# maksimt/rri_nmf

Hardware: AMD Instinct MI355X
Metric: RRI sweeps/sec and achieved HBM GB/s on dense X (n x d, rank k) (higher is better)
Workload: dtype f64

## Files before the change

rri_nmf_amd/csrc/rri_hip.hip:

```cpp
#include <hip/hip_runtime.h>
#include <dlfcn.h>
#include <rccl/rccl.h>

#include <algorithm>
#include <atomic>
#include <chrono>
#include <cmath>
#include <cstdarg>
#include <cstdio>
#include <mutex>
#include <cstdlib>
#include <cstring>
#include <string>
#include <utility>
#include <vector>

#include "rri_hip.h"
#include "rri_layout.hpp"
#include "rri_pick.hpp"
#include "rri_kernels.hpp"
#include "rri_wrri_kernels.hpp"
#include "rri_sparse_kernels.hpp"
#include "rri_onchip_kernels.hpp"

// ... 857 lines not shown
            return;
        }
        const size_t sh = resid_shmem(c);
        flavour([&](auto mk, auto we) {
            hipLaunchKernelGGL((k_resid<SX, mk, we>), dim3(nb), dim3(256), sh, c->stream, (const SX*)c->X, c->ldx, M, ldm, Mbits, ldb,
                               (const double*)c->W, c->ldw, (const double*)c->T, c->LD, (int)c->n, (int)c->d, c->k, rowobj, rowpos, E,
                               c->LD, resid_w_resident(c) ? 1 : 0, xscale(c));
        });
    }
    static void reset_row(rri_ctx* c) {
        if constexpr (!RO) {
            if (c->sparse) {
                (void)hipMemsetAsync(c->xraw, 0, (size_t)c->LD * sizeof(double), c->stream);
                hipLaunchKernelGGL((k_sp_reset_row<SX>), dim3((unsigned)std::max(1, (c->sp_max_row + 255) / 256)), dim3(256), 0,
                                   c->stream, (const i64*)c->sp_rowptr, (const int*)c->sp_col, (const SX*)c->sp_x,
                                   (const double*)c->W, c->ldw, (const double*)c->T, c->LD, c->k, (const i64*)c->itmp,
                                   c->xraw);
                if (c->sparse_x && c->uni_n > 0)
                    hipLaunchKernelGGL(k_spu_reset_row, dim3((unsigned)((c->d + 255) / 256)), dim3(256), 0, c->stream,
                                       (const int*)c->uni_rows, (int)c->uni_n, c->uni_value, (const double*)c->W, c->ldw,
                                       (const double*)c->T, c->LD, c->d, c->k, (const i64*)c->itmp, c->xraw);
                return;
            }
        }
        hipLaunchKernelGGL((k_reset_row<SX>), dim3((unsigned)((c->d + 255) / 256)), dim3(256), 0, c->stream,
                           (const SX*)c->X, c->ldx, (const double*)c->W, c->ldw, (const double*)c->T, c->LD,
                           (int)c->d, c->k, (const i64*)c->itmp, c->xraw, xscale(c));
    }
    static hipError_t set_attrs(const rri_ctx* c) {
        hipError_t e = allow_lds<k_resid<SX, false, false>>(c, 160 * 1024);
        if constexpr (!RO) {
            if (e == hipSuccess) e = allow_lds<k_resid<SX, true, true>>(c, 160 * 1024);
            if (e == hipSuccess) e = allow_lds<k_resid<SX, true, false>>(c, 160 * 1024);
            if (e == hipSuccess) e = allow_lds<k_resid<SX, false, true>>(c, 160 * 1024);
            if (e == hipSuccess) e = allow_lds<k_spx_pass<SX>>(c, SP_BLOCK_BYTES + 64);
        }
        return e;
    }
};

#define DISPATCH(c, expr)                       \
    do {                                        \
        if ((c)->dtype == RRI_F32) {            \
            typedef LaunchX<float> L;           \
            expr;                               \
        } else if ((c)->dtype == RRI_F64) {     \
            typedef LaunchX<double> L;          \
            expr;                               \
        } else {                                \
            f16_unreachable(c);                 \
        }                                       \
    } while (0)
#define DISPATCH_RO(c, expr)                    \
    do {                                        \
        if ((c)->dtype == RRI_F32) {            \
            typedef LaunchX<float> L;           \
            expr;                               \
        } else if ((c)->dtype == RRI_F64) {     \
            typedef LaunchX<double> L;          \
            expr;                               \
        } else if ((c)->dtype == RRI_F16) {     \
            typedef LaunchX<_Float16> L;        \
            expr;                               \
        } else {                                \
            typedef LaunchX<unsigned char> L;   \
            expr;                               \
        }                                       \
    } while (0)

struct LK {
    static int gpart_rows(const rri_ctx* c) { return c->gpart_n; }
    template <bool UPDATE>
    static void wcol_resid(rri_ctx* c, int t, int tn, int sweep) {
        TimedScope ts(c, 1);
        hipLaunchKernelGGL((k_wcol_resid<UPDATE>), dim3(c->nwb256), dim3(256), 0, c->stream, c->W, c->ldw, (int)c->n,
                           c->k, t, tn, (const double*)c->Ypart, c->npanels, (const double*)c->Ttpart, c->nsplit,
                           c->dwv, c->Gpart, sweep, kparams(c), c->st);
        c->gpart_n = c->nwb256;
    }
    static size_t wcol_shmem(const rri_ctx* c) { return (size_t)(2 * c->k + 2 + 256 + 64) * sizeof(double); }
    template <bool UPDATE, bool CARRY>
    static void wcol_src(rri_ctx* c, int t, int tn, int sweep, const double* ypart, int nslices) {
        TimedScope ts(c, 1);
        hipLaunchKernelGGL((k_wcol<UPDATE, CARRY>), dim3(c->nwb), dim3(256), wcol_shmem(c), c->stream, c->W, c->ldw,
                           (int)c->n, c->k, t, tn, ypart, nslices, (const double*)c->Ttpart, c->ttpart_n, c->Gpart,
                           c->XYpart + (i64)t * c->xy_stride, sweep, kparams(c), c->st);
        c->gpart_n = c->nwb;
        if (UPDATE) note_xy(c, t, c->nwb * WCOL_TILES);
    }
    static void note_xy(rri_ctx* c, int t, int rows) {
        if (t == 0) { c->xy_run = 1; c->xy_rows = rows; }
        else c->xy_run = (c->xy_run == t && c->xy_rows == rows) ? t + 1 : -1;
        c->xy_valid = c->xy_run == c->k;
    }
    template <bool UPDATE, bool CARRY>
    static void wcol(rri_ctx* c, int t, int tn, int sweep) {
        wcol_src<UPDATE, CARRY>(c, t, tn, sweep, (const double*)c->Ypart, c->npanels);
    }
    static void reduce(rri_ctx* c) {
        const int nb = (int)((c->LD + 31) / 32) + GRAM_SLICES;
        hipLaunchKernelGGL(k_reduce, dim3(nb), dim3(1024), 0, c->stream, (const double*)c->Zpart, c->LD, c->nrb,
                           (const double*)c->Gpart, gpart_rows(c), c->k, c->red, (const DevState*)c->st);
    }
    static bool light(const rri_ctx* c) { return !(c->prm.project_T_each_iter && c->prm.has_t_row_sum); }
    static void trow(rri_ctx* c, int t, int check_prev, int tprev, int sweep, bool force_final) {
        hipLaunchKernelGGL(k_trow_numer, dim3(c->ntb), dim3(128), 0, c->stream, c->T, c->LD, (int)c->d, c->k, t,
                           (const double*)c->red, c->LD, c->xraw, c->tpart, c->tpart_idx, check_prev, tprev, sweep,
                           kparams(c), c->st, resid_sched(c) ? 1 : 0, resid_sched(c) ? c->told : (double*)nullptr);
        c->tpart_n = c->ntb;
        trow_final_if_needed(c, t, sweep, force_final);
    }
    static bool small(const rri_ctx* c) { return rri::trow_small(gpart_rows(c), c->k, c->ntb32); }
    static void trow_small(rri_ctx* c, int t, int check_prev, int tprev, int sweep, bool force_final) {
        hipLaunchKernelGGL(k_trow_small, dim3(c->ntb32), dim3(1024), 0, c->stream, c->T, c->LD, (int)c->d, c->k, t,
                           (const double*)c->Zpart, c->nrb, (const double*)c->Gpart, gpart_rows(c), c->red, c->LD, c->xraw,
                           c->tpart, c->tpart_idx, check_prev, tprev, sweep, kparams(c), c->st, resid_sched(c) ? 1 : 0,
                           resid_sched(c) ? c->told : (double*)nullptr);
        c->tpart_n = c->ntb32;
        trow_final_if_needed(c, t, sweep, force_final);
    }
    static void trow_final_if_needed(rri_ctx* c, int t, int sweep, bool force_final) {
        if (!light(c) || force_final)
            hipLaunchKernelGGL(k_trow_final, dim3(1), dim3(1024), 0, c->stream, c->T, c->LD, (int)c->d, t, c->xraw,
                               (const double*)c->tpart, (const i64*)c->tpart_idx, c->tpart_n, sweep, kparams(c), c->st);
    }
    static void check_prev_only(rri_ctx* c, int tprev, int sweep, int pos) {
        hipLaunchKernelGGL(k_check_red, dim3(1), dim3(64), 0, c->stream, (const double*)c->red, c->LD, c->k, tprev,
                           sweep, pos, kparams(c), c->st);
    }
    static void tgram(rri_ctx* c, int t, int finish, int sweep) {
        c->ttpart_n = c->nsplit;
        hipLaunchKernelGGL(k_tgram, dim3(c->k, c->nsplit), dim3(256), 0, c->stream, (const double*)c->T, c->LD,
                           (int)c->d, c->k, t, c->Ttpart, (const double*)c->tpart, c->tpart_n, finish, sweep,
                           kparams(c), c->st);
    }
    static void scale_wcol(rri_ctx* c, int t) {
        hipLaunchKernelGGL(k_scale_wcol, dim3((unsigned)((c->n + 255) / 256)), dim3(256), 0, c->stream, c->W,
                           c->ldw, (int)c->n, t, (const DevState*)c->st);
    }
    static void check_wcol(rri_ctx* c, int tprev, int sweep, int pos) {
        hipLaunchKernelGGL(k_check_wcol, dim3(1), dim3(256), 0, c->stream, (const double*)c->Gpart, gpart_rows(c), c->k,
                           tprev, sweep, pos, kparams(c), c->st);
    }
    static void proj_rows(rri_ctx* c, double s, const double* svec) {
        hipLaunchKernelGGL(k_proj_rows, dim3((unsigned)((c->n + 255) / 256)), dim3(256), 0, c->stream, c->W, c->ldw, (int)c->n, c->k, s,
                           svec);
    }
    static void norms(rri_ctx* c, const double* A, i64 rows, i64 cols, i64 ld) {
        hipLaunchKernelGGL(k_norms, dim3(256), dim3(256), 0, c->stream, A, rows, cols, ld, c->normpart);
    }
    static void reset_commit(rri_ctx* c, int t) {
        const i64 m = std::max(c->n, c->d);
        hipLaunchKernelGGL(k_reset_commit, dim3((unsigned)((m + 255) / 256)), dim3(256), 0, c->stream, c->W, c->ldw,
                           c->T, c->LD, (int)c->n, (int)c->d, t, (const i64*)c->itmp, (const double*)c->xraw);
    }
    static void set_row_col(rri_ctx* c, int t, const double* trow, const double* wcolv) {
        const i64 m = std::max(c->n, c->d);
        hipLaunchKernelGGL(k_set_row_col, dim3((unsigned)((m + 255) / 256)), dim3(256), 0, c->stream, c->W, c->ldw,
                           c->T, c->LD, (int)c->n, (int)c->d, t, trow, wcolv);
    }
    static void argmax_rows(rri_ctx* c, int* out) {
        hipLaunchKernelGGL(k_argmax_rows, dim3((unsigned)((c->n + 255) / 256)), dim3(256), 0, c->stream,
                           (const double*)c->W, c->ldw, (int)c->n, c->k, out);
    }
    static void masked_sqerr(rri_ctx* c, const i64* ij, const double* vals, i64 count, double lo, double hi) {
        hipLaunchKernelGGL(k_masked_sqerr, dim3(256), dim3(256), 0, c->stream, (const double*)c->W, c->ldw,
                           (const double*)c->T, c->LD, c->k, ij, vals, count, lo, hi, c->normpart);
    }
};

void launch_convert(rri_ctx* c, int src_dtype, int dst_dtype, bool transpose, const void* src, i64 lds_, void* dst, i64 ldd,
                    i64 rows, i64 cols) {
    const i64 total = rows * cols;
    const unsigned nb = (unsigned)std::min<i64>(4096, (total + 255) / 256);
    pick_type<float, double>(src_dtype, [&](auto s) {
        typedef typename decltype(s)::type Src;
        pick_type<float, double>(dst_dtype, [&](auto d) {
            typedef typename decltype(d)::type Dst;
            pick_bool(transpose, [&](auto tr) {
                hipLaunchKernelGGL((k_convert2d<Src, Dst, tr>), dim3(nb ? nb : 1), dim3(256), 0, c->stream, (const Src*)src,
                                   lds_, (Dst*)dst, ldd, rows, cols);
            });
        });
    });
}

rri_status to_device_half(rri_ctx* c, const void* host, i64 ld, int host_dtype, void* dev, i64 ldd, i64 rows, i64 cols,
                          bool transpose) {
    if (transpose) return fail(c, RRI_ERR_INVALID, "float16 storage is for X only");
    const size_t hs = dtype_size(host_dtype);
    const i64 total = rows * cols;
    const unsigned nb = (unsigned)std::max<i64>(1, std::min<i64>(4096, (total + 255) / 256));
    DevTmp tmp, part;
    HIPCHK(c, tmp.alloc((size_t)rows * cols * hs));
    HIPCHK(c, part.alloc((size_t)nb * 3 * sizeof(double)));
// ... 739 lines not shown
    c->xy_valid = whole_last;
    c->obj_track_pending = a.track != 0;
    return true;
}

void enqueue_from(rri_ctx* c, Cursor cur) {
    if (cur.sweep < c->run_total && onchip_ok(c) && enqueue_onchip(c, cur)) return;
    if (c->until.active && cur.sweep < c->run_total) c->run_total = cur.sweep + 1;
    enqueue_range(c, cur, c->run_total);
    flush_wcheck(c, c->run_total, 0);
}

rri_status read_state(rri_ctx* c, DevState* out) {
    HIPCHK(c, hipMemcpyAsync(out, c->st, sizeof(DevState), hipMemcpyDeviceToHost, c->stream));
    HIPCHK(c, hipStreamSynchronize(c->stream));
    if (c->comm_status != RRI_OK) {
        const rri_status r = c->comm_status;
        c->comm_status = RRI_OK;
        changed(c, CH_ENDED);
        return r;
    }
    return RRI_OK;
}

rri_status status_from_halt(rri_ctx* c, const DevState& s, int32_t* sweeps_done) {
    if (s.halt == 0) {
        c->paused = false;
        if (sweeps_done) *sweeps_done = c->run_total;
        return RRI_OK;
    }
    changed(c, CH_ENDED);
    if (s.halt == HALT_EVENT_STOP) {
        c->paused = false;
        if (sweeps_done) *sweeps_done = s.halt_sweep;
        return RRI_OK;
    }
    if (s.halt > 0) {
        if (c->until.active) c->run_total = std::min(c->run_total, (s.halt == HALT_EVENT_RESET_W && s.halt_pos == 0) ? s.halt_sweep : s.halt_sweep + 1);
        c->paused = true;
        c->pending.kind = s.halt == HALT_EVENT_RESET_T ? RRI_EVENT_RESET_T : RRI_EVENT_RESET_W;
        c->pending.topic = s.halt_topic;
        c->pending.sweep = s.halt_sweep;
        c->pending.resume_topic = s.halt_pos;
        if (s.halt == HALT_EVENT_RESET_T) c->resume_at = Cursor{s.halt_sweep, s.halt_topic, 1};
        else c->resume_at = Cursor{s.halt_sweep, s.halt_pos, 0};
        if (sweeps_done) *sweeps_done = s.halt_sweep;
        return RRI_PAUSED;
    }
    c->paused = false;
    if (sweeps_done) *sweeps_done = s.halt_sweep;
    switch (s.halt) {
        case HALT_ERR_UNBOUNDED:
            return fail(c, RRI_ERR_UNBOUNDED, "Minimum objective is unbounded (topic %d)", s.halt_topic);
        case HALT_ERR_W_COL_ZERO:
            return fail(c, RRI_ERR_W_COL_ZERO, "W[:, t] sums to 0 (topic %d)", s.halt_topic);
        case HALT_ERR_NOT_IMPLEMENTED:
            return fail(c, RRI_ERR_NOT_IMPLEMENTED, "s=%g is not yet implemented", c->prm.t_row_sum);
        case HALT_ERR_GRID_SYNC:
            return fail(c, RRI_ERR_HIP, "the persistent sweep's workgroups could not synchronise (not all resident); RRI_ONCHIP=0 selects the launch-per-phase schedule");
        default:
            return fail(c, RRI_ERR_INVALID, "unknown device status %d", s.halt);
    }
}

rri_status clear_halt(rri_ctx* c) {
    HIPCHK(c, hipMemsetAsync(c->st, 0, 32, c->stream));
    return RRI_OK;
}

rri_switches read_switches() {
    rri_switches sw;
    if (const char* e = getenv("RRI_ONCHIP")) sw.onchip = atoi(e) != 0;
    if (const char* e = getenv("RRI_ONCHIP_OBJ")) sw.onchip_obj = atoi(e) != 0;
    if (const char* e = getenv("RRI_WSWEEP")) sw.wsweep = atoi(e) != 0;
    if (const char* e = getenv("RRI_OBJ_DIRECT")) sw.obj_direct = atoi(e) != 0;
    if (const char* e = getenv("RRI_WMCORR_COLS")) sw.wmcorr_cols = atoi(e) != 0;
    if (const char* e = getenv("RRI_WNW_MASK")) sw.wnw_mask = atoi(e) != 0;
    if (const char* e = getenv("RRI_PASS_ROT")) sw.pass_rot = atoi(e) & 7;
    if (const char* e = getenv("RRI_ROT_CAL")) sw.rot_cal = std::max(0, atoi(e));
    sw.rot_debug = getenv("RRI_ROT_DEBUG") != nullptr;
    if (const char* e = getenv("RRI_MASK_BITS")) sw.mask_bits = atoi(e) != 0;
    if (const char* e = getenv("RRI_PASS_CACHE_MB")) sw.pass_cache_mb = std::max(0.0, atof(e));
    if (const char* e = getenv("RRI_X_PACK")) sw.x_pack = atoi(e) != 0;
    if (const char* e = getenv("RRI_PASS_PK_GEOM")) {
        char* end = nullptr;
        sw.pk_rows = (int)std::min<long>(std::max<long>(0, strtol(e, &end, 10)), 1 << 20);
        sw.pk_il = (end && *end == 'i') ? 1 : (end && *end == 'c') ? 0 : -1;
    }
    return sw;
}

const char* sparse_data_refusal(const rri_ctx* c) {
    return c->sparse_x ? "an RRI_UNWEIGHTED_SPARSE handle keeps X as CSR: it takes its data through rri_upload_X_csr only "
                         "(no dense X, no device binding, no mask)"
                       : "a sparse-pattern handle takes its data through rri_upload_observed_csr";
}

#define REFUSE_RO(c, what)                                                                                              \
    if (ro_store((c)->dtype))                                                                                           \
        return fail((c), RRI_ERR_UNSUPPORTED, "%s is not available on an %s handle (%s stores a dense X that is only read)", what, \
                    dtype_name((c)->dtype), (c)->dtype == RRI_F16 ? "float16" : "uint8")

rri_status ready(rri_ctx* c) {
    if (!c->have_X || !c->have_W || !c->have_T || !c->have_params)
        return fail(c, RRI_ERR_INVALID, "X, W, T and params must be set before stepping");
    if (c->weighted && !c->have_M) return fail(c, RRI_ERR_INVALID, "weighted handle without a mask");
    return RRI_OK;
}

}

extern "C" {

uint32_t rri_abi_version(void) { return RRI_ABI_VERSION; }

const char* rri_last_error(const rri_ctx* ctx) { return ctx ? ctx->err.c_str() : g_create_error.c_str(); }

rri_status rri_create(rri_ctx** out, int64_t n, int64_t d, int32_t k, int32_t dtype, int32_t weighted,
                      int32_t device, void* stream) {
    if (!out) return RRI_ERR_INVALID;
    *out = nullptr;
    if (n < 1 || d < 1 || k < 1) return fail(nullptr, RRI_ERR_INVALID, "need n,d,k >= 1 (got %lld,%lld,%d)", n, d, k);
    if (dtype != RRI_F32 && dtype != RRI_F64 && dtype != RRI_F16 && dtype != RRI_U8)
        return fail(nullptr, RRI_ERR_INVALID, "dtype must be RRI_F32, RRI_F64, RRI_F16 or RRI_U8");
    if (n > 2000000000LL || d > 2000000000LL) return fail(nullptr, RRI_ERR_INVALID, "n, d must fit int32");
    if (k > RRI_MAX_K) return fail(nullptr, RRI_ERR_UNSUPPORTED, "k=%d is above the rank limit RRI_MAX_K = %d of the device path", k, RRI_MAX_K);
    int ndev = 0;
    if (hipGetDeviceCount(&ndev) != hipSuccess || ndev < 1)
        return fail(nullptr, RRI_ERR_HIP, "no HIP device available (librri_hip needs an MI355X)");
    if (device < 0 || device >= ndev) return fail(nullptr, RRI_ERR_INVALID, "device %d out of range [0,%d)", device, ndev);
    if (weighted < 0 || weighted > 4)
        return fail(nullptr, RRI_ERR_INVALID, "weighted must be RRI_UNWEIGHTED, RRI_WEIGHTED_DENSE, RRI_WEIGHTED_SPARSE, "
                                              "RRI_UNWEIGHTED_RESIDUAL or RRI_UNWEIGHTED_SPARSE");
    if (ro_store(dtype) && weighted != RRI_UNWEIGHTED) {
        static const struct { int dtype; const char *stores, *rewritten, *csr; } refusal[] = {
            {RRI_U8, "RRI_U8 stores read-only dense counts (RRI_UNWEIGHTED)", "keeps a stored residual, which counts 0..255 cannot hold",
             "keeps its values in a CSR store, which has no uint8 layout"},
            {RRI_F16, "RRI_F16 stores a read-only dense X (RRI_UNWEIGHTED)",
             "rewrites its stored residual at every topic step, which float16 would round every time",
             "keeps its values in a CSR store, which has no float16 layout"}};
        static const char* const flavour[] = {"", "RRI_WEIGHTED_DENSE", "RRI_WEIGHTED_SPARSE", "RRI_UNWEIGHTED_RESIDUAL", "RRI_UNWEIGHTED_SPARSE"};
        const bool rewritten = weighted == RRI_WEIGHTED_DENSE || weighted == RRI_UNWEIGHTED_RESIDUAL;
        for (const auto& r : refusal)
            if (r.dtype == dtype)
                return fail(nullptr, RRI_ERR_UNSUPPORTED, "%s; %s %s", r.stores, flavour[weighted], rewritten ? r.rewritten : r.csr);
    }
    rri_ctx* c = new rri_ctx();
    c->device = device;
#define CR(call)                                                                                   \
    do {                                                                                           \
        hipError_t e_ = (call);                                                                    \
        if (e_ != hipSuccess) {                                                                    \
            fail(nullptr, RRI_ERR_HIP, "%s failed: %s", #call, hipGetErrorString(e_));             \
            rri_destroy(c);                                                                        \
            return RRI_ERR_HIP;                                                                    \
        }                                                                                          \
    } while (0)
    CR(hipSetDevice(device));
    CR(hipDeviceGetAttribute(&c->n_cu, hipDeviceAttributeMultiprocessorCount, device));
    if (stream) c->stream = (hipStream_t)stream;
    else { CR(hipStreamCreateWithFlags(&c->stream, hipStreamNonBlocking)); c->own_stream = true; }

    c->sw = read_switches();
    const DensePlan p = c->plan = dense_plan(n, d, k, dtype, weighted, c->sw, c->n_cu);
    const bool explicit_resid = p.explicit_resid;
    weighted = p.weighted;
// ... 1865 lines not shown
```

rri_nmf_amd/csrc/rri_kernels.hpp:

```cpp
#pragma once
#include <type_traits>

#include "rri_device.hpp"
#include "rri_halt.hpp"
#include "rri_hip.h"
#include "rri_layout.hpp"
#include "rri_xpack.hpp"

namespace rri {

typedef float f32x4 __attribute__((ext_vector_type(4)));
typedef double f64x2 __attribute__((ext_vector_type(2)));
typedef unsigned u32x4 __attribute__((ext_vector_type(4)));

template <typename SX> struct XVec;
template <> struct XVec<float> {
    typedef f32x4 type;
    static constexpr int N = 4;
    static __device__ __forceinline__ void unpack(const f32x4& v, double (&o)[4]) {
        o[0] = (double)v[0]; o[1] = (double)v[1]; o[2] = (double)v[2]; o[3] = (double)v[3];
    }
    static __device__ __forceinline__ f32x4 pack(const double (&o)[4]) {
        return f32x4{(float)o[0], (float)o[1], (float)o[2], (float)o[3]};
    }
// ... 391 lines not shown
                for (int e = 0; e < VN; ++e) acc[v][e] = fma(wv, xe[e], acc[v][e]);
            }
        }
    }
    if (ok) {
#pragma unroll
        for (int v = 0; v < NV; ++v)
#pragma unroll
            for (int e = 0; e < VN; ++e) {
                if constexpr (XSCALED<SX>) Zmulti[((i64)v * nrb + rb) * ldz + col + e] = acc[v][e] * xs.col[col + e];
                else Zmulti[((i64)v * nrb + rb) * ldz + col + e] = acc[v][e];
            }
    }
}

template <typename SX>
__global__ __launch_bounds__(256) void k_col_count(const SX* __restrict__ X, i64 ldx, int n, int ncols,
                                                   double* __restrict__ Zpart, i64 ldz, int rpb, int npg) {
    typedef XVec<SX> XV;
    typedef typename XV::type V;
    constexpr int VN = XV::N;
    constexpr int PW = 64 * VN;
    const int lane = threadIdx.x & 63, wave = threadIdx.x >> 6;
    const int pg = blockIdx.x % npg, rb = blockIdx.x / npg;
    const int row0 = rb * rpb, row1 = min(n, row0 + rpb);
    const int col = (pg * 4 + wave) * PW + lane * VN;
    if (col >= ncols) return;
    double acc[VN];
#pragma unroll
    for (int e = 0; e < VN; ++e) acc[e] = 0.0;
    for (int r = row0; r < row1; r += 4) {
        V x[4];
#pragma unroll
        for (int u = 0; u < 4; ++u)
            x[u] = (r + u < row1) ? stream_load<true>(reinterpret_cast<const V*>(X + (i64)(r + u) * ldx + col)) : XV::zero();
#pragma unroll
        for (int u = 0; u < 4; ++u) {
            double xe[VN];
            XV::unpack(x[u], xe);
#pragma unroll
            for (int e = 0; e < VN; ++e) acc[e] += xe[e] > 0.0 ? 1.0 : 0.0;
        }
    }
#pragma unroll
    for (int e = 0; e < VN; ++e) Zpart[(i64)rb * ldz + col + e] = acc[e];
}

__global__ __launch_bounds__(256) void k_row_inverse(const double* __restrict__ Ypart, int npanels, int n,
                                                     double* __restrict__ inv) {
    const i64 i = (i64)blockIdx.x * 256 + threadIdx.x;
    if (i >= n) return;
    double xs = 0.0;
    xs = ordered_sum<8>(Ypart + i, n, 0, npanels, 1);
    xs += 2.220446049250313e-16;
    inv[i] = xs < 1e-10 ? -1.0 : 1.0 / xs;
}

template <typename SX>
__global__ __launch_bounds__(256) void k_scale2d(SX* __restrict__ X, i64 ldx, i64 n, int d, const double* __restrict__ s,
                                                 const double* __restrict__ inv) {
    typedef XVec<SX> XV;
    typedef typename XV::type V;
    constexpr int VN = XV::N;
    const i64 vpr = ldx / VN, total = n * vpr;
    const double uniform = 1.0 / (double)d;
    for (i64 v = (i64)blockIdx.x * 256 + threadIdx.x; v < total; v += (i64)gridDim.x * 256) {
        const i64 i = v / vpr;
        const int j = (int)(v - i * vpr) * VN;
        V* p = reinterpret_cast<V*>(X + i * ldx + j);
        double xe[VN];
        XV::unpack(__builtin_nontemporal_load(p), xe);
        const double r = inv ? inv[i] : 1.0;
#pragma unroll
        for (int e = 0; e < VN; ++e) {
            if (j + e >= d) { xe[e] = 0.0; continue; }
            const double t = s ? xe[e] * s[j + e] : xe[e];
            xe[e] = r < 0.0 ? uniform : r * t;
        }
        __builtin_nontemporal_store(XV::pack(xe), p);
    }
}


template <bool UPDATE, bool CARRY>
__global__ __launch_bounds__(256) void k_wcol(double* __restrict__ Wt, i64 ldw, int n, int k, int t, int tn,
                                              const double* __restrict__ Ypart, int npanels,
                                              const double* __restrict__ Ttpart, int nsplit,
                                              double* __restrict__ Gpart, double* __restrict__ xyp, int sweep,
                                              KParams p, DevState* st) {
    if (st->halt) return;
    const int tid = threadIdx.x, lane = tid & 63, wave = tid >> 6;
    extern __shared__ __attribute__((aligned(16))) unsigned char smem[];
    double* tts = reinterpret_cast<double*>(smem);
    double* gsh = tts + k;
    double* dsh = gsh + k + 2;
    double* wsh = dsh + 256;
    double cden = 0.0;
    int mode = 0;
    for (int l = tid; l < k + 2; l += 256) gsh[l] = 0.0;
    if (UPDATE) {
        for (int l = tid; l < k; l += 256) {
            tts[l] = ordered_sum<8>(Ttpart + l, k, 0, nsplit, 1);
        }
        __syncthreads();
        cden = tts[t] + p.reg_w_l2;
        __syncthreads();
        if (tid == 0) tts[t] = 0.0;
        mode = wcol_denominator_mode(cden, p);
        if (mode < 0) {
            if (blockIdx.x == 0 && tid == 0) halt_set(st, mode, t, sweep, t);
            return;
        }
    }
    __syncthreads();
    constexpr int CH = 16;
    constexpr int TILES = WCOL_TILES;
    for (int tile = 0; tile < TILES; ++tile) {
        const i64 i = ((i64)blockIdx.x * TILES + tile) * 64 + lane;
        if (((i64)blockIdx.x * TILES + tile) * 64 >= n) break;
        const bool valid = i < n;
        const double wn = (CARRY && valid) ? Wt[(i64)tn * ldw + i] : 0.0;
        double y = 0.0;
        if (UPDATE && wave == 0 && valid) y = ordered_sum<8>(Ypart + i, n, 0, npanels, 1);
        double dotv = 0.0;
        for (int l0 = wave; l0 < k; l0 += 4 * CH) {
            double wl[CH];
#pragma unroll
            for (int q = 0; q < CH; ++q) {
                const int l = l0 + 4 * q;
                wl[q] = (l < k && valid && !(UPDATE && l == t)) ? Wt[(i64)l * ldw + i] : 0.0;
            }
#pragma unroll
            for (int q = 0; q < CH; ++q) {
                const int l = l0 + 4 * q;
                if (l < k) {
                    if (UPDATE) dotv = fma(wl[q], tts[l], dotv);
                    if (CARRY && !(UPDATE && l == t)) {
                        const double g = wave_sum<double>(wn * wl[q]);
                        if (lane == 0) gsh[l] += g;
                    }
                }
            }
        }
        double wnew = 0.0;
        if (UPDATE) {
            dsh[wave * 64 + lane] = dotv;
            __syncthreads();
            if (wave == 0) {
                const double dot = (dsh[lane] + dsh[64 + lane]) + (dsh[128 + lane] + dsh[192 + lane]);
                if (valid) {
                    const double numer = (y - dot) - p.reg_w_l1;
                    if (mode == 0) wnew = fmax(numer, 0.0) / (cden + p.eps);
                    else wnew = (-numer + cden < 0.0) ? p.w_row_sum : 0.0;
                    Wt[(i64)t * ldw + i] = wnew;
                }
                wsh[lane] = wnew;
            }
            __syncthreads();
            wnew = wsh[lane];
        }
        if (wave == 0) {
            const double nwp = wave_sum<double>(wn * wn);
            const double swp = wave_sum<double>(wnew);
            if (lane == 0) { gsh[k] += nwp; gsh[k + 1] += swp; }
            if (UPDATE) {
                const double xy = wave_sum<double>(wnew * y);
                if (lane == 0) xyp[(i64)blockIdx.x * TILES + tile] = xy;
            }
        } else if (wave == 1 && UPDATE && CARRY) {
            const double gt = wave_sum<double>(wn * wnew);
            if (lane == 0) gsh[t] += gt;
        }
        if (UPDATE) __syncthreads();
    }
    __syncthreads();
    double* gp = Gpart + (i64)blockIdx.x * (k + 2);
    for (int l = tid; l < k + 2; l += 256) gp[l] = gsh[l];
}

__host__ __device__ constexpr int wsweep_kp(int k) { return (k + 3) & ~3; }
__host__ __device__ constexpr size_t wsweep_lds_bytes(int k) { return ((size_t)k * wsweep_kp(k) + 64 * (size_t)k) * sizeof(double); }

__global__ __launch_bounds__(64) void k_wsweep_rows(double* __restrict__ Wt, double* __restrict__ Wprev, i64 ldw, int n, int k,
                                                    int t0, const double* __restrict__ Qt, const double* __restrict__ G,
                                                    double* __restrict__ colsum, int nwb, double* __restrict__ xyp,
                                                    i64 xy_stride, KParams p, const DevState* __restrict__ st) {
    if (st->halt) return;
    extern __shared__ __attribute__((aligned(16))) unsigned char smem[];
    const int kp = wsweep_kp(k);
    double* gsh = reinterpret_cast<double*>(smem);
    double* wsh = gsh + (size_t)k * kp;
    const int lane = threadIdx.x;
    const i64 i = (i64)blockIdx.x * 64 + lane;
    const bool valid = i < n;
    for (int q = lane; q < k * kp; q += 64) {
        const int l = q / kp, c = q - l * kp;
        gsh[q] = c < k ? G[(i64)l * k + c] : 0.0;
    }
    constexpr int CH = 8;
    for (int l0 = 0; l0 < k; l0 += CH) {
        double wv[CH];
#pragma unroll
        for (int q = 0; q < CH; ++q) wv[q] = (l0 + q < k && valid) ? Wt[(i64)(l0 + q) * ldw + i] : 0.0;
#pragma unroll
        for (int q = 0; q < CH; ++q) {
            const int l = l0 + q;
// ... 116 lines not shown
    if (st->halt) return;
    __shared__ double scratch[40];
    const i64 i = (i64)blockIdx.x * 256 + threadIdx.x;
    double cden = 1.0, nt = 0.0;
    int mode = 0;
    if (UPDATE) {
        nt = ordered_sum<8>(Ttpart + t, k, 0, nsplit, 1);
        cden = nt + p.reg_w_l2;
        mode = wcol_denominator_mode(cden, p);
        if (mode < 0) {
            if (blockIdx.x == 0 && threadIdx.x == 0) halt_set(st, mode, t, sweep, t);
            return;
        }
    }
    double wnew = 0.0, dwi = 0.0, wn = 0.0;
    if (i < n) {
        if (UPDATE) {
            const double y = ordered_sum<8>(Ypart + i, n, 0, npanels, 1);
            const double w0 = Wt[(i64)t * ldw + i];
            const double numer = fma(w0, nt, y) - p.reg_w_l1;
            if (mode == 0) wnew = fmax(numer, 0.0) / (cden + p.eps);
            else wnew = (-numer + cden < 0.0) ? p.w_row_sum : 0.0;
            Wt[(i64)t * ldw + i] = wnew;
            dwi = wnew - w0;
            dw[i] = dwi;
        }
        wn = (UPDATE && tn == t) ? wnew : Wt[(i64)tn * ldw + i];
    }
    const double g = block_sum(wn * dwi, scratch);
    const double nwp = block_sum(wn * wn, scratch);
    const double sw = block_sum(wnew, scratch);
    double* gp = Gpart + (i64)blockIdx.x * (k + 2);
    for (int l = threadIdx.x; l < k + 2; l += 256) gp[l] = (l == t && UPDATE) ? g : (l == k ? nwp : (l == k + 1 ? sw : 0.0));
}

__global__ __launch_bounds__(1024) void k_reduce(const double* __restrict__ Zpart, i64 ldz, int nrb,
                                                 const double* __restrict__ Gpart, int nwb, int k,
                                                 double* __restrict__ red, const DevState* __restrict__ st) {
    if (st->halt) return;
    __shared__ double sh[32 * 33];
    const int tid = threadIdx.x;
    const int ngram = Gpart ? GRAM_SLICES : 0;
    const int nzb = gridDim.x - ngram;
    if ((int)blockIdx.x < nzb) {
        const int c = tid & 31, g = tid >> 5;
        const i64 j = (i64)blockIdx.x * 32 + c;
        double a = 0.0;
        if (j < ldz) a = ordered_sum<8>(Zpart + j, ldz, g, nrb, 32);
        sh[g * 33 + c] = a;
        __syncthreads();
        if (tid < 32 && j < ldz) {
            double s = 0.0;
            for (int q = 0; q < 32; ++q) s += sh[q * 33 + tid];
            red[j] = s;
        }
    } else {
        const int gs = blockIdx.x - nzb;
        const int per = (nwb + GRAM_SLICES - 1) / GRAM_SLICES;
        const int b0 = gs * per, b1 = min(nwb, b0 + per);
        const int lane = tid & 63, wave = tid >> 6;
        for (int l0 = 0; l0 < k + 2; l0 += 64) {
            const int l = l0 + lane;
            double a = 0.0;
            if (l < k + 2) a = ordered_sum<8>(Gpart + l, k + 2, b0 + wave, b1, 16);
            __syncthreads();
            sh[wave * 64 + lane] = a;
            __syncthreads();
            if (wave == 0 && l < k + 2) {
                double s = 0.0;
                for (int q = 0; q < 16; ++q) s += sh[q * 64 + lane];
                red[ldz + (i64)gs * (k + 2) + l] = s;
            }
        }
    }
}

__device__ __forceinline__ double red_gram(const double* __restrict__ red, i64 ldz, int k, int l) {
    double s = 0.0;
#pragma unroll
    for (int g = 0; g < GRAM_SLICES; ++g) s += red[ldz + (i64)g * (k + 2) + l];
    return s;
}

__global__ __launch_bounds__(128) void k_trow_numer(double* __restrict__ T, i64 ldt, int d, int k, int t,
                                                    const double* __restrict__ red, i64 ldz,
                                                    double* __restrict__ xraw, double* __restrict__ tpart,
                                                    i64* __restrict__ tpart_idx, int check_prev, int tprev,
                                                    int sweep, KParams p, DevState* st, int resid_form,
                                                    double* __restrict__ told) {
    if (st->halt) return;
    const int tid = threadIdx.x;
    __shared__ double scratch[40];
    __shared__ double gsh[RRI_MAX_K];
    const double nw = red_gram(red, ldz, k, k);
    if (check_prev) {
        const int code = wcol_code(red_gram(red, ldz, k, k + 1), p);
        if (code != 0) {
            if (blockIdx.x == 0 && tid == 0) halt_set(st, code, tprev, sweep, t);
            return;
        }
    }
    const double c = nw + p.reg_t_l2;
    const bool project = p.project_T && p.has_trs;
    const int mode = trow_denominator_mode(c, p);
    if (mode < 0) {
        if (blockIdx.x == 0 && tid == 0) halt_set(st, mode, t, sweep, t);
        return;
    }
    for (int l = tid; l < k; l += 128) gsh[l] = (l == t) ? (resid_form ? -nw : 0.0) : red_gram(red, ldz, k, l);
    __syncthreads();
    const i64 j = (i64)blockIdx.x * 128 + tid;
    double x = 0.0, mx = -1.0e300;
    if (j < d) {
        if (told) told[j] = T[(i64)t * ldt + j];
        double a0 = 0.0, a1 = 0.0, a2 = 0.0, a3 = 0.0;
        for (int l0 = 0; l0 < k; l0 += 16) {
            double tv[16];
#pragma unroll
            for (int q = 0; q < 16; ++q) tv[q] = (l0 + q < k) ? T[(i64)(l0 + q) * ldt + j] : 0.0;
#pragma unroll
            for (int q = 0; q < 16; q += 4) {
                if (l0 + q < k) a0 = fma(gsh[l0 + q], tv[q], a0);
                if (l0 + q + 1 < k) a1 = fma(gsh[l0 + q + 1], tv[q + 1], a1);
                if (l0 + q + 2 < k) a2 = fma(gsh[l0 + q + 2], tv[q + 2], a2);
                if (l0 + q + 3 < k) a3 = fma(gsh[l0 + q + 3], tv[q + 3], a3);
            }
        }
        const double acc = (a0 + a1) + (a2 + a3);
        const double numer = (red[j] - acc) - p.reg_t_l1;
        if (mode == 0) x = fmax(numer, 0.0) / (c + p.eps);
        else if (mode == 1) x = (-numer + c < 0.0) ? p.t_row_sum : 0.0;
        else { x = numer; mx = numer; }
        xraw[j] = x;
        if (mode == 1 || (mode == 0 && !project)) T[(i64)t * ldt + j] = x;
    }
    if (mode != 2) {
        const double s = block_sum(x, scratch);
        if (tid == 0) tpart[blockIdx.x] = s;
    } else {
        i64 idx = (j < d) ? j : (i64)0x7fffffffffffffffLL;
        wave_argmax(mx, idx);
        __shared__ double wm[2];
        __shared__ i64 wi[2];
        if ((tid & 63) == 0) { wm[tid >> 6] = mx; wi[tid >> 6] = idx; }
        __syncthreads();
        if (tid == 0) {
            if (wm[1] > wm[0] || (wm[1] == wm[0] && wi[1] < wi[0])) { wm[0] = wm[1]; wi[0] = wi[1]; }
            tpart[blockIdx.x] = wm[0];
            tpart_idx[blockIdx.x] = wi[0];
        }
    }
    if (blockIdx.x == 0 && tid == 0) st->tmode = mode;
}

__global__ __launch_bounds__(1024) void k_trow_small(double* __restrict__ T, i64 ldt, int d, int k, int t,
                                                     const double* __restrict__ Zpart, int nrb,
                                                     const double* __restrict__ Gpart, int nwb, double* __restrict__ red,
                                                     i64 ldz, double* __restrict__ xraw, double* __restrict__ tpart,
                                                     i64* __restrict__ tpart_idx, int check_prev, int tprev, int sweep,
                                                     KParams p, DevState* st, int resid_form, double* __restrict__ told) {
    if (st->halt) return;
    const int tid = threadIdx.x;
    __shared__ double sh[32 * 33];
    __shared__ double gsh[RRI_MAX_K + 2];
    __shared__ double zs[32];
    const int cc = tid & 31, g = tid >> 5;
    const i64 j = (i64)blockIdx.x * 32 + cc;
    constexpr int ZB = 16;
    double zpre[ZB];
#pragma unroll
    for (int q = 0; q < ZB; ++q) {
        const int r = g + 32 * q;
        zpre[q] = (j < ldz && r < nrb) ? Zpart[(i64)r * ldz + j] : 0.0;
    }
    double tkeep[4];
#pragma unroll
    for (int q = 0; q < 4; ++q) {
        const int l = g + 32 * q;
        tkeep[q] = (j < d && l < k && (l != t || resid_form)) ? T[(i64)l * ldt + j] : 0.0;
    }
    for (int l0 = 0; l0 < k + 2; l0 += 32) {
        const int l = l0 + cc;
        double a = 0.0;
        if (l < k + 2) a = ordered_sum<8>(Gpart + l, k + 2, g, nwb, 32);
        __syncthreads();
        sh[g * 33 + cc] = a;
        __syncthreads();
        if (tid < 32 && l < k + 2) {
            double s = 0.0;
            for (int q = 0; q < 32; ++q) s += sh[q * 33 + tid];
            gsh[l] = s;
        }
    }
    __syncthreads();
    const double nw = gsh[k];
    if (check_prev) {
        const int code = wcol_code(gsh[k + 1], p);
        if (code != 0) {
            if (blockIdx.x == 0 && tid == 0) halt_set(st, code, tprev, sweep, t);
            return;
        }
    }
    const double c = nw + p.reg_t_l2;
    const bool project = p.project_T && p.has_trs;
    const int mode = trow_denominator_mode(c, p);
    if (mode < 0) {
        if (blockIdx.x == 0 && tid == 0) halt_set(st, mode, t, sweep, t);
        return;
    }
    if (blockIdx.x == 0)
        for (int i = tid; i < GRAM_SLICES * (k + 2); i += 1024) red[ldz + i] = i < k + 2 ? gsh[i] : 0.0;
    {
        double a = 0.0;
#pragma unroll
        for (int q = 0; q < ZB; ++q) a += zpre[q];
        if (j < ldz) a = ordered_sum_acc<8>(a, Zpart + j, ldz, g + 32 * ZB, nrb, 32);
        sh[g * 33 + cc] = a;
    }
    __syncthreads();
    if (tid < 32) {
        double s = 0.0;
        for (int q = 0; q < 32; ++q) s += sh[q * 33 + tid];
        zs[tid] = s;
        if (j < ldz) red[j] = s;
    }
    __syncthreads();
    {
// ... 901 lines not shown
```

rri_nmf_amd/csrc/rri_layout.hpp:

```cpp
#pragma once
#include <algorithm>
#include <cstdint>
#include <string>
#include <vector>

#include "rri_hip.h"

namespace rri {

typedef long long i64;
inline i64 round_up(i64 a, i64 b) { return (a + b - 1) / b * b; }

constexpr size_t dtype_size(int dt) { return dt == RRI_F32 ? 4 : dt == RRI_F64 ? 8 : dt == RRI_F16 ? 2 : dt == RRI_U8 ? 1 : 0; }
constexpr int load_elems(int dt) { return dt == RRI_U8 ? 8 : dtype_size(dt) ? (int)(16 / dtype_size(dt)) : 0; }
constexpr int load_bytes(int dt) { return load_elems(dt) * (int)dtype_size(dt); }

constexpr int WCOL_TILES = 1;
constexpr int GRAM_SLICES = RRI_GRAM_SLICES;
constexpr int TG_ROWS = 32;
constexpr int SP_BLOCK_BYTES = 120 * 1024;
constexpr i64 spx_block_cap() { return (i64)(SP_BLOCK_BYTES / 8 - 64) / 64 * 64; }
struct SpWork { int blk, s0, s1, pad; };
constexpr int ONCHIP_THREADS = 512, ONCHIP_WAVES = ONCHIP_THREADS / 64;
constexpr int ONCHIP_SMALL_K = 22;
constexpr int ONCHIP_MAX_K = 64;
constexpr int ONCHIP_CWA = 32;
constexpr int ONCHIP_PG = ONCHIP_THREADS / ONCHIP_CWA;

constexpr double PASS_CACHE_MB = 256.0;
constexpr int PK_ROWS_MAX = 512;

struct rri_switches {
    bool onchip = true;
    bool onchip_obj = true;
    bool wsweep = true;
    bool obj_direct = false;
    bool wmcorr_cols = true;
    bool wnw_mask = true;
    int pass_rot = -1;
    int rot_cal = 1;
    bool rot_debug = false;
    bool mask_bits = true;
    double pass_cache_mb = PASS_CACHE_MB;
    int pk_rows = 0;
    int pk_il = -1;
    int x_pack = -1;
};

struct SpDims { int nblk = 1, bw = 1; i64 nseg = 0, gdim = 0; };
inline SpDims sp_dims(i64 n, i64 d, int which, bool sparse_x, size_t es) {
    const i64 block_bytes = SP_BLOCK_BYTES;
    const i64 cap = sparse_x ? std::min<i64>(spx_block_cap(), std::max<i64>(64, (block_bytes / 8 - 64) / 64 * 64))
                             : block_bytes / (3 * (i64)es);
    SpDims s;
    s.gdim = which == 0 ? d : n;
    s.nseg = which == 0 ? n : d;
    s.nblk = (int)((s.gdim + cap - 1) / cap);
    s.bw = (int)round_up((s.gdim + s.nblk - 1) / s.nblk, 64);
    return s;
}
inline int sp_target_items(int n_cu, bool sparse_x) { return std::max(1, sparse_x ? n_cu / 2 : n_cu); }

inline bool ro_pass_interleaved(int ro_il, int npanels, int nrb) { return ro_il >= 0 ? ro_il != 0 : npanels * nrb <= 1024; }
inline bool wtrow_small(bool has_comm, int nrb) { return !has_comm && nrb <= 64; }

struct DensePlan {
    i64 n = 0, d = 0, LD = 0;
    int k = 0, dtype = RRI_F32, weighted = 0;
    bool explicit_resid = false, sparse_x = false, sparse = false;
    int VN = 4, PW = 1024, kp = 8;
    int npanels = 1, rpb = 1, nrb = 1, nwb = 1, nwb256 = 1, ntb = 1, ntb32 = 1, nsplit = 4;
    i64 red_elems = 0;
    int ro_il = -1;
    int cpart_rows = 0;
    i64 gpart_rows = 1, ttpart_rows = 1, tpart_rows = 1;
    int xy_stride = 1;
    SpDims sp[2];
};

inline DensePlan dense_plan(i64 n, i64 d, int k, int dtype, int flavour, const rri_switches& sw, int n_cu) {
    DensePlan p;
    p.explicit_resid = flavour == RRI_UNWEIGHTED_RESIDUAL;
    p.sparse_x = flavour == RRI_UNWEIGHTED_SPARSE;
    const int weighted = (p.explicit_resid || p.sparse_x) ? (int)RRI_UNWEIGHTED : flavour;
    const bool explicit_resid = p.explicit_resid;
    p.n = n; p.d = d; p.k = k; p.dtype = dtype; p.weighted = weighted;
    p.sparse = weighted == RRI_WEIGHTED_SPARSE || p.sparse_x;
    p.kp = (int)round_up(k, 8);
    p.VN = load_elems(dtype);
    p.PW = 64 * p.VN * 4;
    p.LD = round_up(d, p.VN);

    p.npanels = (int)((p.LD + p.PW - 1) / p.PW);
    const i64 rpb_cap = ((40 * 1024 - 4 * 8 * 72 * 8) / ((weighted ? 11 : explicit_resid ? 7 : 5) * 8)) / 16 * 16;
    i64 rpb = 0;
    {
        const bool rmw = explicit_resid || weighted == RRI_WEIGHTED_DENSE;
        const int total_max = weighted == RRI_WEIGHTED_DENSE ? 16384 : rmw ? 8192 : 1024;
        const i64 rows_min = weighted == RRI_WEIGHTED_DENSE ? 48 : rmw ? 96 : 192;
        for (int total = total_max; total >= 512 && rpb == 0; total -= 512) {
            const int nrb_t = std::max(1, total / p.npanels);
            const i64 r = (n + nrb_t - 1) / nrb_t;
            if (r >= rows_min || total == 512) rpb = r;
        }
    }
    rpb = std::max<i64>(rpb, 32);
    rpb = std::min<i64>(round_up(rpb, 16), rpb_cap);
    if (dtype == RRI_F32 && !weighted && !explicit_resid && !p.sparse) {
        rpb = sw.pk_rows > 0 ? std::min<i64>(round_up(std::max(sw.pk_rows, 16), 16), rpb_cap) : std::min<i64>(rpb, PK_ROWS_MAX);
        if (sw.pk_rows > 0) p.ro_il = sw.pk_il;
    }
    p.rpb = (int)rpb;
    p.nrb = (int)((n + rpb - 1) / rpb);
    if (p.sparse) {
        for (int w = 0; w < 2; ++w) p.sp[w] = sp_dims(n, d, w, p.sparse_x, dtype_size(dtype));
        p.npanels = p.sp[0].nblk;
        p.nrb = p.sp[1].nblk;
    }
    p.nwb = (int)((n + 64 * WCOL_TILES - 1) / (64 * WCOL_TILES));
    p.nwb256 = (int)((n + 255) / 256);
    p.ntb = (int)((d + 127) / 128);
    p.ntb32 = (int)((p.LD + 31) / 32);
    p.nsplit = (int)std::max<i64>(1, std::min<i64>(8, d / 2048));
    p.red_elems = round_up(std::max<i64>(p.LD + (i64)GRAM_SLICES * (k + 2), weighted ? 2 * p.LD + 2 : 0), 4);
    p.gpart_rows = std::max(p.nwb, p.nrb);
    p.xy_stride = (int)std::max<i64>(std::max<i64>(p.gpart_rows, (i64)p.nwb * WCOL_TILES), (i64)std::max(n_cu, 1));
    p.ttpart_rows = std::max(p.nsplit, p.ntb32);
    p.tpart_rows = std::max(p.ntb, p.ntb32);
    if (weighted && !p.sparse) p.cpart_rows = (int)std::max<i64>(256, (n + 2047) / 2048);
// ... 222 lines not shown
```

Before: 33.89.

## Split trow topic dot across four wave groups and widen wcol Ypart reduction

The T-row numerator kernel gains a G=4 variant that splits the k-topic dot product across four 128-thread groups, strided by l mod 4. Each group prefetches its first T tile before the grid-level checks, and the partials are combined through shared memory. k_wcol also gets a template parameter for the ordered_sum batch width, using 16 when there are 9-16 Y slices. The aim is to hide the latency of the serial per-column T reads with more parallelism, at the cost of larger blocks and an extra shared-memory reduction. Both paths are on by default and can be disabled with new environment switches; a switch to turn off trow_small is added too.

```diff
diff --git a/rri_nmf_amd/csrc/rri_hip.hip b/rri_nmf_amd/csrc/rri_hip.hip
--- a/rri_nmf_amd/csrc/rri_hip.hip
+++ b/rri_nmf_amd/csrc/rri_hip.hip
@@ -963,9 +963,12 @@
     template <bool UPDATE, bool CARRY>
     static void wcol_src(rri_ctx* c, int t, int tn, int sweep, const double* ypart, int nslices) {
         TimedScope ts(c, 1);
-        hipLaunchKernelGGL((k_wcol<UPDATE, CARRY>), dim3(c->nwb), dim3(256), wcol_shmem(c), c->stream, c->W, c->ldw,
-                           (int)c->n, c->k, t, tn, ypart, nslices, (const double*)c->Ttpart, c->ttpart_n, c->Gpart,
-                           c->XYpart + (i64)t * c->xy_stride, sweep, kparams(c), c->st);
+        pick_int<16, 8>(UPDATE && c->sw.step_trips && nslices > 8 && nslices <= 16 ? 16 : 8, [&](auto yb) {
+            if constexpr (UPDATE || yb == 8)
+                hipLaunchKernelGGL((k_wcol<UPDATE, CARRY, yb>), dim3(c->nwb), dim3(256), wcol_shmem(c), c->stream, c->W, c->ldw,
+                                   (int)c->n, c->k, t, tn, ypart, nslices, (const double*)c->Ttpart, c->ttpart_n, c->Gpart,
+                                   c->XYpart + (i64)t * c->xy_stride, sweep, kparams(c), c->st);
+        });
         c->gpart_n = c->nwb;
         if (UPDATE) note_xy(c, t, c->nwb * WCOL_TILES);
     }
@@ -985,13 +988,15 @@
     }
     static bool light(const rri_ctx* c) { return !(c->prm.project_T_each_iter && c->prm.has_t_row_sum); }
     static void trow(rri_ctx* c, int t, int check_prev, int tprev, int sweep, bool force_final) {
-        hipLaunchKernelGGL(k_trow_numer, dim3(c->ntb), dim3(128), 0, c->stream, c->T, c->LD, (int)c->d, c->k, t,
-                           (const double*)c->red, c->LD, c->xraw, c->tpart, c->tpart_idx, check_prev, tprev, sweep,
-                           kparams(c), c->st, resid_sched(c) ? 1 : 0, resid_sched(c) ? c->told : (double*)nullptr);
+        pick_int<4, 1>(c->sw.step_trips ? 4 : 1, [&](auto G) {
+            hipLaunchKernelGGL((k_trow_numer<G>), dim3(c->ntb), dim3(128 * G), 0, c->stream, c->T, c->LD, (int)c->d, c->k, t,
+                               (const double*)c->red, c->LD, c->xraw, c->tpart, c->tpart_idx, check_prev, tprev, sweep,
+                               kparams(c), c->st, resid_sched(c) ? 1 : 0, resid_sched(c) ? c->told : (double*)nullptr);
+        });
         c->tpart_n = c->ntb;
         trow_final_if_needed(c, t, sweep, force_final);
     }
-    static bool small(const rri_ctx* c) { return rri::trow_small(gpart_rows(c), c->k, c->ntb32); }
+    static bool small(const rri_ctx* c) { return c->sw.trow_small && rri::trow_small(gpart_rows(c), c->k, c->ntb32); }
     static void trow_small(rri_ctx* c, int t, int check_prev, int tprev, int sweep, bool force_final) {
         hipLaunchKernelGGL(k_trow_small, dim3(c->ntb32), dim3(1024), 0, c->stream, c->T, c->LD, (int)c->d, c->k, t,
                            (const double*)c->Zpart, c->nrb, (const double*)c->Gpart, gpart_rows(c), c->red, c->LD, c->xraw,
@@ -1897,6 +1902,8 @@
     if (const char* e = getenv("RRI_MASK_BITS")) sw.mask_bits = atoi(e) != 0;
     if (const char* e = getenv("RRI_PASS_CACHE_MB")) sw.pass_cache_mb = std::max(0.0, atof(e));
     if (const char* e = getenv("RRI_X_PACK")) sw.x_pack = atoi(e) != 0;
+    if (const char* e = getenv("RRI_TROW_SMALL")) sw.trow_small = atoi(e) != 0;
+    if (const char* e = getenv("RRI_STEP_TRIPS")) sw.step_trips = atoi(e) != 0;
     if (const char* e = getenv("RRI_PASS_PK_GEOM")) {
         char* end = nullptr;
         sw.pk_rows = (int)std::min<long>(std::max<long>(0, strtol(e, &end, 10)), 1 << 20);
diff --git a/rri_nmf_amd/csrc/rri_kernels.hpp b/rri_nmf_amd/csrc/rri_kernels.hpp
--- a/rri_nmf_amd/csrc/rri_kernels.hpp
+++ b/rri_nmf_amd/csrc/rri_kernels.hpp
@@ -497,7 +497,7 @@
 }
 
 
-template <bool UPDATE, bool CARRY>
+template <bool UPDATE, bool CARRY, int YB = 8>
 __global__ __launch_bounds__(256) void k_wcol(double* __restrict__ Wt, i64 ldw, int n, int k, int t, int tn,
                                               const double* __restrict__ Ypart, int npanels,
                                               const double* __restrict__ Ttpart, int nsplit,
@@ -536,7 +536,7 @@
         const bool valid = i < n;
         const double wn = (CARRY && valid) ? Wt[(i64)tn * ldw + i] : 0.0;
         double y = 0.0;
-        if (UPDATE && wave == 0 && valid) y = ordered_sum<8>(Ypart + i, n, 0, npanels, 1);
+        if (UPDATE && wave == 0 && valid) y = ordered_sum<YB>(Ypart + i, n, 0, npanels, 1);
         double dotv = 0.0;
         for (int l0 = wave; l0 < k; l0 += 4 * CH) {
             double wl[CH];
@@ -819,16 +819,35 @@
     return s;
 }
 
-__global__ __launch_bounds__(128) void k_trow_numer(double* __restrict__ T, i64 ldt, int d, int k, int t,
-                                                    const double* __restrict__ red, i64 ldz,
-                                                    double* __restrict__ xraw, double* __restrict__ tpart,
-                                                    i64* __restrict__ tpart_idx, int check_prev, int tprev,
-                                                    int sweep, KParams p, DevState* st, int resid_form,
-                                                    double* __restrict__ told) {
+template <int G>
+__global__ __launch_bounds__(128 * G, G == 1 ? 1 : 7) void k_trow_numer(double* __restrict__ T, i64 ldt, int d, int k, int t,
+                                                        const double* __restrict__ red, i64 ldz,
+                                                        double* __restrict__ xraw, double* __restrict__ tpart,
+                                                        i64* __restrict__ tpart_idx, int check_prev, int tprev,
+                                                        int sweep, KParams p, DevState* st, int resid_form,
+                                                        double* __restrict__ told) {
+    static_assert(G == 1 || G == 4, "the topics are split as the four accumulators are: l mod 4");
     if (st->halt) return;
     const int tid = threadIdx.x;
+    const int ct = G == 1 ? tid : (tid & 127);
+    const int grp = G == 1 ? 0 : __builtin_amdgcn_readfirstlane(tid >> 7);
+    const i64 j = (i64)blockIdx.x * 128 + ct;
     __shared__ double scratch[40];
     __shared__ double gsh[RRI_MAX_K];
+    __shared__ double psh[G > 1 ? (G - 1) * 128 : 1];
+    double tv[16];
+    double rj = 0.0, tj = 0.0;
+    if constexpr (G > 1) {
+#pragma unroll
+        for (int q = 0; q < 16; ++q) {
+            const int l = grp + 4 * q;
+            tv[q] = (j < d && l < k) ? T[(i64)l * ldt + j] : 0.0;
+        }
+        if (grp == 0 && j < d) {
+            rj = red[j];
+            if (told) tj = T[(i64)t * ldt + j];
+        }
+    }
     const double nw = red_gram(red, ldz, k, k);
     if (check_prev) {
         const int code = wcol_code(red_gram(red, ldz, k, k + 1), p);
@@ -844,42 +863,74 @@
         if (blockIdx.x == 0 && tid == 0) halt_set(st, mode, t, sweep, t);
         return;
     }
-    for (int l = tid; l < k; l += 128) gsh[l] = (l == t) ? (resid_form ? -nw : 0.0) : red_gram(red, ldz, k, l);
+    for (int l = tid; l < k; l += 128 * G) gsh[l] = (l == t) ? (resid_form ? -nw : 0.0) : red_gram(red, ldz, k, l);
     __syncthreads();
-    const i64 j = (i64)blockIdx.x * 128 + tid;
     double x = 0.0, mx = -1.0e300;
-    if (j < d) {
-        if (told) told[j] = T[(i64)t * ldt + j];
-        double a0 = 0.0, a1 = 0.0, a2 = 0.0, a3 = 0.0;
-        for (int l0 = 0; l0 < k; l0 += 16) {
-            double tv[16];
-#pragma unroll
-            for (int q = 0; q < 16; ++q) tv[q] = (l0 + q < k) ? T[(i64)(l0 + q) * ldt + j] : 0.0;
-#pragma unroll
-            for (int q = 0; q < 16; q += 4) {
-                if (l0 + q < k) a0 = fma(gsh[l0 + q], tv[q], a0);
-                if (l0 + q + 1 < k) a1 = fma(gsh[l0 + q + 1], tv[q + 1], a1);
-                if (l0 + q + 2 < k) a2 = fma(gsh[l0 + q + 2], tv[q + 2], a2);
-                if (l0 + q + 3 < k) a3 = fma(gsh[l0 + q + 3], tv[q + 3], a3);
-            }
-        }
-        const double acc = (a0 + a1) + (a2 + a3);
-        const double numer = (red[j] - acc) - p.reg_t_l1;
-        if (mode == 0) x = fmax(numer, 0.0) / (c + p.eps);
-        else if (mode == 1) x = (-numer + c < 0.0) ? p.t_row_sum : 0.0;
-        else { x = numer; mx = numer; }
-        xraw[j] = x;
-        if (mode == 1 || (mode == 0 && !project)) T[(i64)t * ldt + j] = x;
+    if constexpr (G == 1) {
+        if (j < d) {
+            if (told) told[j] = T[(i64)t * ldt + j];
+            double a0 = 0.0, a1 = 0.0, a2 = 0.0, a3 = 0.0;
+            for (int l0 = 0; l0 < k; l0 += 16) {
+#pragma unroll
+                for (int q = 0; q < 16; ++q) tv[q] = (l0 + q < k) ? T[(i64)(l0 + q) * ldt + j] : 0.0;
+#pragma unroll
+                for (int q = 0; q < 16; q += 4) {
+                    if (l0 + q < k) a0 = fma(gsh[l0 + q], tv[q], a0);
+                    if (l0 + q + 1 < k) a1 = fma(gsh[l0 + q + 1], tv[q + 1], a1);
+                    if (l0 + q + 2 < k) a2 = fma(gsh[l0 + q + 2], tv[q + 2], a2);
+                    if (l0 + q + 3 < k) a3 = fma(gsh[l0 + q + 3], tv[q + 3], a3);
+                }
+            }
+            const double acc = (a0 + a1) + (a2 + a3);
+            const double numer = (red[j] - acc) - p.reg_t_l1;
+            if (mode == 0) x = fmax(numer, 0.0) / (c + p.eps);
+            else if (mode == 1) x = (-numer + c < 0.0) ? p.t_row_sum : 0.0;
+            else { x = numer; mx = numer; }
+            xraw[j] = x;
+            if (mode == 1 || (mode == 0 && !project)) T[(i64)t * ldt + j] = x;
+        }
+    } else {
+        double a = 0.0;
+        for (int l0 = grp; l0 < k; l0 += 64) {
+            if (l0 != grp) {
+#pragma unroll
+                for (int q = 0; q < 16; ++q) tv[q] = (j < d && l0 + 4 * q < k) ? T[(i64)(l0 + 4 * q) * ldt + j] : 0.0;
+            }
+#pragma unroll
+            for (int q = 0; q < 16; ++q)
+                if (l0 + 4 * q < k) a = fma(gsh[l0 + 4 * q], tv[q], a);
+        }
+        if (grp > 0) psh[(grp - 1) * 128 + ct] = a;
+        __syncthreads();
+        if (grp == 0 && j < d) {
+            if (told) told[j] = tj;
+            const double acc = (a + psh[ct]) + (psh[128 + ct] + psh[256 + ct]);
+            const double numer = (rj - acc) - p.reg_t_l1;
+            if (mode == 0) x = fmax(numer, 0.0) / (c + p.eps);
+            else if (mode == 1) x = (-numer + c < 0.0) ? p.t_row_sum : 0.0;
+            else { x = numer; mx = numer; }
+            xraw[j] = x;
+            if (mode == 1 || (mode == 0 && !project)) T[(i64)t * ldt + j] = x;
+        }
     }
     if (mode != 2) {
-        const double s = block_sum(x, scratch);
+        double s;
+        if constexpr (G == 1) s = block_sum(x, scratch);
+        else {
+            const double w = wave_sum<double>(x);
+            if ((tid & 63) == 0 && tid < 128) scratch[tid >> 6] = w;
+            __syncthreads();
+            s = 0.0;
+            s += scratch[0];
+            s += scratch[1];
+        }
         if (tid == 0) tpart[blockIdx.x] = s;
     } else {
-        i64 idx = (j < d) ? j : (i64)0x7fffffffffffffffLL;
+        i64 idx = (grp == 0 && j < d) ? j : (i64)0x7fffffffffffffffLL;
         wave_argmax(mx, idx);
         __shared__ double wm[2];
         __shared__ i64 wi[2];
-        if ((tid & 63) == 0) { wm[tid >> 6] = mx; wi[tid >> 6] = idx; }
+        if ((tid & 63) == 0 && tid < 128) { wm[tid >> 6] = mx; wi[tid >> 6] = idx; }
         __syncthreads();
         if (tid == 0) {
             if (wm[1] > wm[0] || (wm[1] == wm[0] && wi[1] < wi[0])) { wm[0] = wm[1]; wi[0] = wi[1]; }
diff --git a/rri_nmf_amd/csrc/rri_layout.hpp b/rri_nmf_amd/csrc/rri_layout.hpp
--- a/rri_nmf_amd/csrc/rri_layout.hpp
+++ b/rri_nmf_amd/csrc/rri_layout.hpp
@@ -45,6 +45,8 @@
     int pk_rows = 0;
     int pk_il = -1;
     int x_pack = -1;
+    bool trow_small = true;
+    bool step_trips = true;
 };
 
 struct SpDims { int nblk = 1, bw = 1; i64 nseg = 0, gdim = 0; };
```

Result: no change. 33.97 (median of 3 runs) (+0.2%).
